# FrancisTheCat/raytracing_c

Hardware: AMD Instinct MI355X
Metric: Mray/s (higher is better)
Workload: dtype f32; 1 GPU; helmet.glb 1920x1080, 256 spp, 8 bounces (BASELINE.json configs[2]); partition=single GPU

## Files before the change

### include/rt_hip_diag.h

```cpp
#ifndef RT_HIP_DIAG_H
#define RT_HIP_DIAG_H

#include "rt_hip.h"

#ifdef __cplusplus
extern "C" {
#endif

extern void rt_diag_set_tokens(void *disney_proc, void *debug_proc, void *background_proc);

extern void rt_diag_multi_fault(i32 no_peer, i32 failing_slot);

extern int  rt_set_pipeline(i32 pipeline);
extern i32  rt_get_pipeline(void);
extern void rt_set_wavefront_capacity(i64 records);

extern int rt_get_ledger(u64 *out, i32 n);
extern int rt_get_wave_times(u64 *out, i32 max_waves);
extern i64 rt_diag_device_bytes_live(void);
extern int rt_diag_release_staging(void);
extern RT_Device_Scene *rt_diag_cached_scene(Scene const *scene);


extern int rt_test_math(i32 op, i32 n, f32 const *x, f32 const *y, f32 *out);
// ... 4 lines not shown
extern int rt_test_encode_sweep(u64 out[260]);
extern int rt_test_group_sum(i32 group, i32 n_waves, u64 const *in, u8 const *valid, u64 *out);
extern int rt_test_sky_add_group(void);
extern int rt_test_node_order(i32 n, u32 const *t_min, u8 const *cand, u32 *out);

extern int rt_test_trace(RT_Device_Scene *dscene, i32 n, f32 const *rays,
                         f32 *out_t, i32 *out_tri, f32 *out_uv);

extern int rt_test_trace_stream(RT_Device_Scene *dscene, i32 n, f32 const *rays, f32 const *pyramid, i32 exit_lanes, i32 mode,
                                f32 *out_t, i32 *out_tri, f32 *out_uv, u64 visits[2]);

extern int rt_test_tile_order(i32 n_tiles, u32 const *cost, u32 *order);

extern int rt_test_texture(RT_Device_Scene *dscene, i32 tex, i32 n, f32 const *uv, f32 *out_rgb);


#define RT_TEST_SHARED_TAPS 4
extern int rt_test_shade(RT_Device_Scene *dscene, i32 mode, i32 n, i32 const *tri, f32 const *in, u32 const *state_in,
                         f32 *out, u32 *state_out, i32 *terminate, i32 *textured);
extern int rt_test_shade_hit(RT_Device_Scene *dscene, i32 mode, i32 max_bounces, i32 n, i32 const *tri, f32 const *hit, f32 const *ray,
                             f32 const *carry, u32 const *state_in, i32 const *bounce_in, f32 *out, u32 *out_words);
extern int rt_test_feature_hit(RT_Device_Scene *dscene, i32 n, i32 const *tri, f32 const *hit, f32 const *ray, f32 *out, i32 *flag);
extern int rt_test_brdf(i32 n, f32 const *params, f32 const *in_dir, u32 const *state_in, f32 *out_dir, f32 *brdf, u32 *state_out);
extern int rt_test_background(RT_Device_Scene *dscene, i32 mode, i32 n, f32 const *dir, f32 *rgb);
extern int rt_test_primary_ray(Camera const *camera, i32 width, i32 height, i32 n, i32 const *xys, f32 *rays);

#ifdef __cplusplus
}
#endif

#endif
```

### raytracing_c_amd/csrc/rt_dev.hip.h

```cpp
#ifndef RT_DEV_HIP_H
#define RT_DEV_HIP_H

#include <hip/hip_runtime.h>
#include <stdint.h>

#include "rt_device.h"
#include "../../include/rt_math.h"

#define RT_BLOCK_WAVES 4
#define RT_BLOCK_THREADS (RT_BLOCK_WAVES * 64)

struct Ray3 {
  rt_v3 o, d;
  float inv_x, inv_y, inv_z;
  bool  fast;
};

__device__ __forceinline__ rt_v3 slab_bias3(const Ray3 &r) {
#ifdef RT_MATH_NO_FMA
  return rt_v3_make(0.0f, 0.0f, 0.0f);
#else
  float px, py, pz;
  asm volatile("v_mul_f32 %0, %1, %2" : "=v"(px) : "v"(r.o.x), "v"(r.inv_x));
  asm volatile("v_mul_f32 %0, %1, %2" : "=v"(py) : "v"(r.o.y), "v"(r.inv_y));
// ... 638 lines not shown
  if (POW24_LDS) p = rt_pow24_poly(b) * *reinterpret_cast<const float *>(reinterpret_cast<const char *>(rt_pow24_lds) + (((uint32_t)as_i(b) >> 21) & 28u));
  else p = rt_pow24_core(b);
  if (!(b >= 0x1p-5f && b < 2.0f)) p = rt_powf(b, 2.4f);
  return p;
#else
  const float b = __builtin_fmaf(r, c, q);
  const float t = __builtin_amdgcn_fmed3f(2.4f * rt_logf(b), -87.0f, 87.0f);
  const float p = rt_expf(t);
  return (b > 0.0f) ? p : 0.0f;
#endif
}
template <bool POW24_LDS = false>
__device__ __forceinline__ rt_v3 srgb_to_linear_tex(rt_v3 v) {
  return rt_v3_make(srgb_to_linear_tex1<POW24_LDS>(v.x), srgb_to_linear_tex1<POW24_LDS>(v.y), srgb_to_linear_tex1<POW24_LDS>(v.z));
}

__device__ __forceinline__ float bg_coord_u(float t) { return rt_madd(t, 1.0f / (2.0f * RT_PI), 0.5f); }
__device__ __forceinline__ float bg_coord_v(float t) { return rt_madd(-t, 1.0f / RT_PI, 0.5f); }
template <class PT>
__device__ __forceinline__ rt_v3 background_lookup(const PT &P, rt_v3 dir) {
  float u = bg_coord_u(atan2_dev(dir.z, dir.x));
  float v = bg_coord_v(asin_dev(dir.y));
  return srgb_to_linear_tex<Pow24InLds<PT>::value>(tex_bilinear<false>(P, P.bg_texture, u, v));
}


__device__ __forceinline__ float pow5(float m) { return m * m * m * m * m; }
__device__ __forceinline__ float luminance(rt_v3 x) { return rt_v3_dot(x, rt_v3_make(0.2126f, 0.7152f, 0.0722f)); }

__device__ __forceinline__ float ggx_D(float roughness, float NoH) {
  float a2 = roughness * roughness;
  float d = rt_madd(NoH * NoH, rt_madd(a2, a2, -1.0f), 1.0f);
  return a2 / (RT_PI * (d * d));
}

__device__ __forceinline__ float smith_G(float NDotV, float alpha2) {
  float a = alpha2 * alpha2;
  float b = NDotV * NDotV;
  return (2.0f * NDotV) / (NDotV + sqrt_dev(rt_madd(-a, b, a + b)));
}

__device__ __forceinline__ rt_v3 cosine_hemisphere(uint32_t &rng) {
  float angle = rt_rand_f32(&rng) * 2.0f * RT_PI;
  float distance = sqrt_dev(rt_rand_f32(&rng));
  float s, c;
  rt_sincosf(angle, &s, &c);
// ... 905 lines not shown
  const RT_DTexture *textures;
  const uint32_t *texels;
  int32_t bg_texture, max_bounces;
};

template <class SPT, class ARGS>
__device__ __forceinline__ void shade_params(SPT &SP, const ARGS A, const bool with_materials) {
  SP.tris = with_materials ? A->tris : nullptr; SP.mats = with_materials ? A->mats : nullptr;
  SP.textures = A->textures; SP.texels = A->texels;
  SP.bg_texture = A->bg_texture; SP.max_bounces = A->max_bounces;
}

struct ShadeParamsLds : ShadeParams {};
template <> struct Pow24InLds<ShadeParamsLds> { static constexpr bool value = RT_MATH_POW24 != 0; };

struct ShadeParamsShared : ShadeParams {};
struct ShadeParamsLdsShared : ShadeParamsLds {};
template <> struct SharedTaps<ShadeParamsShared> { static constexpr bool value = true; };
template <> struct SharedTaps<ShadeParamsLdsShared> { static constexpr bool value = true; };
template <> struct Pow24InLds<ShadeParamsLdsShared> { static constexpr bool value = RT_MATH_POW24 != 0; };
template <bool SHARED_TAPS> struct PathShadeParams { typedef ShadeParamsLds type; };
template <> struct PathShadeParams<true> { typedef ShadeParamsLdsShared type; };

struct PrimaryParams {
  float cam[3][4];
  float focal_length, inv_width, inv_height, aspect;
};
template <class CAM, class ARGS>
__device__ __forceinline__ void primary_params(PrimaryParams &PP, const CAM S, const ARGS A) {
#pragma unroll
  for (int i = 0; i < 3; i++)
#pragma unroll
    for (int j = 0; j < 4; j++) PP.cam[i][j] = S->cam[i][j];
  PP.focal_length = S->focal_length; PP.inv_width = A->inv_width; PP.inv_height = A->inv_height; PP.aspect = A->aspect;
}

#include "rt_tile.hip.h"

#endif
```

### raytracing_c_amd/csrc/rt_device.h

```cpp
#ifndef RT_DEVICE_H
#define RT_DEVICE_H

#include <stdint.h>

#define RT_NODE_F4   12
#define RT_LEAF_F4   18
#define RT_TRI_F4     7
#define RT_MAT_F4     9
#define RT_MAT_FLOATS 36
#define RT_MAX_DEPTH  8

#define RT_LDS_BYTES            (160 * 1024)
#define RT_LDS_NODE_BYTES       208
#define RT_LDS_TABLE_BYTES      64
#define RT_LDS_PERM_LEVEL_BYTES 256
#define RT_LDS_ACC_TILE_BYTES   1536

#define RT_MAT_DISNEY 0
#define RT_MAT_DEBUG  1

#define RT_TILE      8
#define RT_TILE_PIX  64

#define RT_PARK_RECORD_DWORDS (18 * 128)
enum {
  RT_CNT_PATHS = 0, RT_CNT_RAYS, RT_CNT_NODES, RT_CNT_LEAVES, RT_CNT_SHADES, RT_CNT_BG, RT_CNT_TEXTURED,
  RT_CNT_SKIPPED_ROOT,
  RT_CNT_LEDGER,
  RT_CNT_LEAFLESS = 136,
  RT_CNT_FUSED_ROOT,
  RT_CNT_TRIANGLELESS,
  RT_N_COUNTERS
};
#define RT_CNT_LEDGER_SLOTS (RT_CNT_LEAFLESS - RT_CNT_LEDGER)



typedef struct {
  uint32_t offset;
  int32_t  width, height, stride;
} RT_DTexture;
#define RT_TEX_TILE_INDEX(x, y, tpr) ((((y) >> 2) * (tpr) + ((x) >> 2)) * 16 + (((y) & 3) << 2) + ((x) & 3))

typedef struct RT_KView {
  float    cam[3][4];
  float    focal_length;
  uint32_t seed;
  uint32_t pad[2];
} RT_KView;

typedef struct {
  const float    *nodes;
  const float    *leaves;
  const float    *tris;
  const float    *mats;
  const RT_DTexture *textures;
  const uint32_t *texels;
  int32_t depth;
  int32_t last_row_offset;
  int32_t bg_texture;
  int32_t n_nodes;
  float cam[3][4];
  float focal_length;
  float inv_width, inv_height, aspect;
  int32_t width, height, samples, max_bounces;
// ... 15 lines not shown
  uint32_t *tile_next;
  uint32_t *open_groups;
  int32_t n_tiles;
  int32_t chunk_shift;
  int32_t n_chunks_tile;
  int32_t n_sample_blocks;
  int32_t drain_thresh;
  int32_t grab_max;
  uint32_t *park;
  int32_t short_div;
  int32_t pyr_nodes;
  uint32_t *wf_hit0;
  uint32_t *wf_hit;
  uint32_t *wf_ray[2];
  uint32_t *wf_cnt_hit0, *wf_cnt_hit, *wf_cnt_ray[2];
  uint32_t *wf_ctl;
  int32_t wf_soft_chunks;
  int32_t wf_bounce;
  int32_t wf_n_waves;
  const RT_KView *views;
  int32_t n_views;
  int32_t tiles_per_view;
  int32_t pixels_per_view;
} RT_KParams;

typedef struct {
  const float *rays;
  const float *t_max;
  float       *hits;
  uint8_t     *flags;
  uint32_t    *head;
  unsigned long long *counters;
  int32_t      n;
  int32_t      grab;
  int32_t      exit_lanes;
} RT_QParams;
enum { RT_QCNT_RAYS = 0, RT_QCNT_HITS, RT_QCNT_NODES, RT_QCNT_LEAVES, RT_QUERY_COUNTERS };
#define RT_HIT_DWORDS     22

typedef struct {
  unsigned long long *sums;
  uint32_t    *head;
  int32_t      n_units;
  int32_t      grab;
  int32_t      tiles_x;
  int32_t      shift;
// ... 39 lines not shown
```

### raytracing_c_amd/csrc/rt_diag.cpp

```cpp

#include "rt_host.h"

#include <cmath>
#include <vector>

#include "../../include/rt_math.h"
#include "../../include/rt_hip_diag.h"

#ifndef RT_DIAG_VARIANTS
#error rt_diag.cpp belongs to the diagnostic library only (-DRT_DIAG_VARIANTS)
#endif

extern "C" {
int rt_launch_test_math(int op, int n, const float *x, const float *y, float *out, hipStream_t stream);
int rt_launch_test_rcp_sweep(unsigned long long *counts, hipStream_t stream);
int rt_launch_test_srgb_sweep(unsigned long long *counts, hipStream_t stream);
int rt_launch_test_env_sweep(int which, uint32_t seed, unsigned long long *counts, hipStream_t stream);
int rt_launch_test_quantize_sweep(unsigned long long *counts, hipStream_t stream);
int rt_launch_test_encode_sweep(unsigned long long *counts, hipStream_t stream);
int rt_launch_test_sky_add_group(void);
int rt_launch_test_group_sum(int group, int n_waves, const unsigned long long *in, const unsigned char *valid, unsigned long long *out,
                              hipStream_t stream);
int rt_launch_test_node_order(int n, const uint32_t *t_min, const unsigned char *cand, uint32_t *out, hipStream_t stream);
int rt_launch_test_trace(const RT_KParams *P, int n, const float *rays, float *out_t, int *out_tri, float *out_uv,
                         hipStream_t stream);
int rt_launch_test_trace_stream(const RT_KParams *P, int n, const float *rays, const float *pyr, int exit_lanes, int n_blocks,
                                int smem_bytes, float *out_t, int *out_tri, float *out_uv, unsigned long long *visits,
                                hipStream_t stream);
int rt_launch_test_texture(const RT_KParams *P, int tex, int n, const float *uv, float *out, hipStream_t stream);
int rt_launch_test_shade(const RT_KParams *P, int lds, int n, const int *tri, const float *in, const uint32_t *state_in, float *out,
                         uint32_t *state_out, int *terminate, int *textured, hipStream_t stream);
int rt_launch_test_shade_hit(const RT_KParams *P, int mode, int n, const int *tri, const float *hit, const float *ray, const float *carry,
                             const uint32_t *state_in, const int *bounce_in, float *out, uint32_t *iout, hipStream_t stream);
int rt_launch_test_feature_hit(const RT_KParams *P, int n, const int *tri, const float *hit, const float *ray, float *out, int *flag,
                               hipStream_t stream);
int rt_launch_test_brdf(int n, const float *params, const float *in_dir, const uint32_t *state_in, float *out_dir, float *brdf,
                        uint32_t *state_out, hipStream_t stream);
int rt_launch_test_background(const RT_KParams *P, int lds, int n, const float *dir, float *rgb, hipStream_t stream);
int rt_launch_test_primary_ray(const RT_KParams *P, int n, const int *xys, float *rays, hipStream_t stream);
int rt_wf_launch_camera(const RT_KParams *P, int n_blocks, int geometry, int smem_bytes, hipStream_t stream);
int rt_wf_launch_trace(const RT_KParams *P, int n_blocks, int geometry, int smem_bytes, hipStream_t stream);
int rt_wf_launch_shade(const RT_KParams *P, int n_blocks, int first, hipStream_t stream);
}

std::atomic<int>            g_pipeline{0};
static std::atomic<int64_t> g_wf_cap_records{(int64_t)96 << 20};

extern "C" int rt_set_pipeline(i32 pipeline) {
  if (pipeline != 0 && pipeline != 1) return rt_fail("rt_set_pipeline: %d is not 0 (tile stream) or 1 (wavefront)", pipeline);
  g_pipeline.store(pipeline);
  return 0;
}
extern "C" i32 rt_get_pipeline(void) { return g_pipeline.load(); }
extern "C" void rt_set_wavefront_capacity(i64 records) {
  if (records >= 1024) g_wf_cap_records.store(records);
}

extern "C" void rt_diag_set_tokens(void *disney, void *debug, void *background) {
  if (disney) g_tok_disney = (Shader_Proc)disney;
  if (debug) g_tok_debug = (Shader_Proc)debug;
  if (background) g_tok_background = (Background_Proc)background;
// ... 479 lines not shown
  if (ensure_device(D) != 0) return -1;
  if (n <= 0 || !params || !in_dir || !state_in || !out_dir || !brdf || !state_out) return rt_fail("rt_test_brdf: bad arguments");
  DevMem<float> dp, di, dout, db;
  DevMem<uint32_t> ds0, ds1;
  HIP_TRY(dp.grow((size_t)n * 8));
  HIP_TRY(di.grow((size_t)n * 3));
  HIP_TRY(dout.grow((size_t)n * 3));
  HIP_TRY(db.grow((size_t)n * 4));
  HIP_TRY(ds0.grow((size_t)n));
  HIP_TRY(ds1.grow((size_t)n));
  HIP_TRY(hipMemcpy(dp, params, (size_t)n * 32, hipMemcpyHostToDevice));
  HIP_TRY(hipMemcpy(di, in_dir, (size_t)n * 12, hipMemcpyHostToDevice));
  HIP_TRY(hipMemcpy(ds0, state_in, (size_t)n * 4, hipMemcpyHostToDevice));
  int rc = rt_launch_test_brdf(n, dp, di, ds0, dout, db, ds1, nullptr);
  if (rc == 0) rc = (int)hipMemcpy(out_dir, dout, (size_t)n * 12, hipMemcpyDeviceToHost);
  if (rc == 0) rc = (int)hipMemcpy(brdf, db, (size_t)n * 16, hipMemcpyDeviceToHost);
  if (rc == 0) rc = (int)hipMemcpy(state_out, ds1, (size_t)n * 4, hipMemcpyDeviceToHost);
  if (rc != 0) return rt_fail("rt_test_brdf failed: %s", hipGetErrorString((hipError_t)rc));
  return 0;
}

extern "C" int rt_test_background(RT_Device_Scene *d, i32 mode, i32 n, f32 const *dir, f32 *rgb) {
  if (!d || n <= 0 || !dir || !rgb) return rt_fail("rt_test_background: bad arguments");
  if (mode != 0 && mode != 1) return rt_fail("rt_test_background: mode %d is not 0 (ShadeParams) or 1 (ShadeParamsLds)", mode);
  if (!all_finite(dir, (size_t)n * 3)) return rt_fail("rt_test_background: non-finite direction");
  Device &D = *d->dev;
  std::lock_guard<std::mutex> lock(D.mutex);
  DeviceGuard guard(D);
  if (ensure_device(D) != 0) return -1;
  RT_KParams K;
  scene_only_kparams(&K, d);
  DevMem<float> dd, dout;
  HIP_TRY(dd.grow((size_t)n * 3));
  HIP_TRY(dout.grow((size_t)n * 3));
  HIP_TRY(hipMemcpy(dd, dir, (size_t)n * 12, hipMemcpyHostToDevice));
  int rc = rt_launch_test_background(&K, mode, n, dd, dout, nullptr);
  if (rc == 0) rc = (int)hipMemcpy(rgb, dout, (size_t)n * 12, hipMemcpyDeviceToHost);
  if (rc != 0) return rt_fail("rt_test_background failed: %s", hipGetErrorString((hipError_t)rc));
  return 0;
}

extern "C" int rt_test_primary_ray(Camera const *camera, i32 width, i32 height, i32 n, i32 const *xys, f32 *rays) {
  Device &D = dev0();
  std::lock_guard<std::mutex> lock(D.mutex);
  if (ensure_device(D) != 0) return -1;
  if (!camera || width < 1 || height < 1 || n <= 0 || !xys || !rays) return rt_fail("rt_test_primary_ray: bad arguments");
  RT_KParams K;
  memset(&K, 0, sizeof K);
// ... 15 lines not shown
```

### raytracing_c_amd/csrc/rt_host.h

```cpp
#pragma once

#include <hip/hip_runtime.h>

#include <algorithm>
#include <atomic>
#include <chrono>
#include <cstdarg>
#include <cstdio>
#include <cstdlib>
#include <cstring>
#include <condition_variable>
#include <mutex>
#include <thread>
#include <unordered_map>
#include <vector>

#include "../../include/rt_hip.h"
#include "rt_device.h"
#include "rt_mem.h"

extern "C" {
int rt_launch_path_kernel(const RT_KParams *P, int n_waves, int smem_bytes, int wg_waves, hipStream_t stream);
int rt_launch_prepare(int n_tiles, uint32_t *tile_next, uint32_t *open_groups, unsigned long long *counters, uint32_t *work_head,
                      uint32_t *cost_cur, const uint32_t *cost_prev, uint32_t *order, hipStream_t stream);
int rt_launch_resolve(int width, int height, int samples, int chunks_x, const int32_t *local_chunks, int n_local_chunks,
                      const unsigned long long *accum, uint8_t *tiles, uint8_t *image, float *linear,
                      hipStream_t stream);
int rt_launch_untile(int width, int height, int chunks_x, int n_chunks, const int32_t *owner_slot,
                     const uint8_t *all_tiles, uint8_t *image, hipStream_t stream);
int rt_launch_lightmap(const RT_KParams *P, const float *verts, int n_tris, int lw, int lh, int stride, int comp,
                       int samples, int *owner, uint8_t *pixels, hipStream_t stream);
int rt_launch_denoise(int width, int height, int src_stride, int src_comp, int dst_stride, int dst_comp,
                      const uint8_t *src, uint8_t *dst, hipStream_t stream);
int rt_launch_pack_texture(const uint8_t *raw, int width, int rows, int y0, int stride, int comp, uint32_t *out,
                           hipStream_t stream);
int rt_launch_query(const RT_KParams *P, const RT_QParams *Q, int any, int wg_waves, int n_blocks, int smem_bytes, hipStream_t stream);
int rt_launch_hit_attributes(const RT_KParams *P, int n, const float *rays, const float *hits, float *out, hipStream_t stream);
int rt_launch_features(const RT_KParams *P, const RT_FParams *F, int n_blocks, int smem_bytes, hipStream_t stream);
int rt_launch_features_resolve(int n_pixels, int samples, const unsigned long long *sums, float *coverage, float *albedo, float *normal,
                               float *position, hipStream_t stream);
int rt_launch_features_motion(const RT_KParams *P, const RT_FParams *F, const float *kept, unsigned long long *motion_sums, int n_blocks,
                              int smem_bytes, hipStream_t stream);
int rt_launch_motion_resolve(int n_pixels, int samples, const unsigned long long *sums, float *motion, hipStream_t stream);
int rt_launch_refit(int len, int depth, int n_internal, const void *d_src, const int *d_source_of_slot, float *d_block, float *d_nodes,
                    float *d_leaves, float *d_tris, unsigned char *d_populated, unsigned int *d_max_edge_bits, hipStream_t stream);
int rt_refit_check(Scene const *scene, Triangle_Slice src, i32 const *slot_of_source, i32 *source_of_slot);
int rt_launch_guided_pack(int n_pixels, int demodulate, RT_Frame frame, void *c0, void *g0, void *g1, hipStream_t stream);
int rt_launch_guided_filter(int width, int height, int step, float k_n, float k_p, float k_c, int last, int demodulate, const void *src,
                            void *dst, const void *g0, const void *g1, RT_Frame frame, float *out, uint8_t *image, hipStream_t stream);
int rt_launch_temporal(const RT_TParams *P, RT_Frame frame, const void *hist_in, void *hist_out, float *out, float *length,
                       uint8_t *image, hipStream_t stream);
int rt_launch_temporal_motion(const RT_TParams *P, RT_Frame frame, const float *motion, const void *hist_in, void *hist_out, float *out,
                              float *length, uint8_t *image, hipStream_t stream);
int rt_launch_temporal_pack(int n_pixels, const float *c, const float *len, const float *cov, const float *n, const float *w, void *hist,
                            hipStream_t stream);
int rt_launch_temporal_unpack(int n_pixels, const void *hist, float *c, float *len, float *cov, float *n, float *w, hipStream_t stream);
int rt_launch_temporal_moments(const RT_TParams *P, RT_Frame frame, const void *hist_in, void *hist_out, float *out, float *length,
                               uint8_t *image, const void *mom_in, void *mom_out, hipStream_t stream);
// ... 275 lines not shown
  DevMem<uint32_t>    tile_next;
  int32_t             tile_next_n = 0;
  DevMem<uint32_t>    park;
  DevMem<uint32_t>    cost[2];
  DevMem<uint32_t>    order;
  int32_t      sched_tiles = 0, sched_cur = 0;
  bool         sched_valid = false;
  uint64_t     sched_key = 0;
  DevMem<RT_KView>    views;
  PinnedMem<RT_KView> views_host;
  DevEvent            views_copied;
  ChunkListStage      list;
};

#pragma GCC visibility pop

struct RT_Device_Scene {
  Device      *dev = nullptr;
  DevMem<float>       nodes, leaves, tris, mats;
  DevMem<float>       kept_leaves;
  bool                has_kept = false;
  DevMem<RT_DTexture> textures;
  DevMem<uint32_t>    texels;
  int32_t      depth = 0, last_row_offset = 0, bg_texture = -1, n_nodes = 0;
  int32_t      n_triangles = 0, n_materials = 0, n_textures = 0;
  int64_t      bytes = 0;
  float        max_edge = 0.0f;
  bool         boxes_ordered = true;
  std::vector<float> mats_host;
  bool         shared_taps = false;
  uint64_t     stamp = 0;
  std::vector<const void *> mat_ptrs;
  std::vector<int32_t>      mat_first_tri;
  std::vector<FpBlock>      fp_blocks;
  uint64_t                  full_fp = 0;
  std::unordered_map<uint64_t, int> mat_map;
  std::vector<const Image *>        tex_sources;
  std::vector<RT_DTexture>          tex_descs;
  LaunchState ls[RT_LAUNCH_STATES + 2];
  DevMem<uint32_t>    wf_hit0, wf_hit, wf_ray[2];
  DevMem<uint32_t>    wf_cnt;
  DevMem<uint32_t>    wf_ctl;
  PinnedMem<uint32_t> wf_ctl_host;
  int64_t             wf_soft0 = 0, wf_hard0 = 0, wf_ray_chunks = 0, wf_hit_chunks = 0;
  int32_t             wf_waves = 0;
};
// ... 94 lines not shown
```

### raytracing_c_amd/csrc/rt_kernels.hip

```cpp

#include "rt_dev.hip.h"


#ifdef RT_LEDGER
#define RT_LEDGER_WAVES 8192
__device__ uint32_t g_ledger[RT_LEDGER_WAVES * RT_LEDGER_ROW];
__global__ void rt_ledger_reduce_kernel(unsigned long long *counters) {
  const int slot = threadIdx.x;
  if (slot >= LG_N || slot >= RT_LEDGER_ROW) return;
  unsigned long long sum = 0ull;
  for (int w = 0; w < RT_LEDGER_WAVES; w++) sum += g_ledger[w * RT_LEDGER_ROW + slot];
  counters[RT_CNT_LEDGER + slot] = sum;
}
#endif

template <int WAVES, bool LDSN, int MIN_WAVES_PER_SIMD, bool SHORT_DIV, bool VIEWS, bool SHARED_TAPS>
__global__ __launch_bounds__(WAVES * 64, MIN_WAVES_PER_SIMD) void rt_path_kernel_stream(RT_KParams P) {
  extern __shared__ float4 smem[];
  const int lane = threadIdx.x & 63;
  const int wave = threadIdx.x >> 6;
  const int n_lds = LDSN ? P.n_lds_nodes : 0;
  const float4 *lds_nodes = smem;
  const WaveLds L = wave_lds(smem, n_lds, P.depth, wave);
  unsigned long long *acc = L.acc;
// ... 80 lines not shown
    LGT1(LG_CYC_TILE);

    int   pix = 0, bounce = 0;
    uint32_t rng = 0;
    Ray3  ray;
    ray_setup(ray, rt_v3_make(0, 0, 0), rt_v3_make(0, 0, 1));
    rt_v3 tint = rt_v3_make(1, 1, 1), emis = rt_v3_make(0, 0, 0);
    TravState T = RT_TRAV_IDLE;

    bool tile_open = true;
    TileUnits U;
    tile_units_init(U, queue_open);
    int  n_parked = 0;
    uint32_t *park = cold_args()->park;

    if ((tile_root_miss || n_list > 0) && cold_args()->max_bounces > 0) {
      RT_KArgs A = cold_args();
      typename CamSrc<VIEWS>::type S;
      if constexpr (VIEWS) S = vrec; else S = A;
      const int width = A->width, height = A->height, sample_first = A->sample_first, sample_end = A->sample_end;
      const uint32_t n_sb = (uint32_t)A->n_sample_blocks, gmax = (uint32_t)A->grab_max;
      PrimaryParams PP;
      primary_params(PP, S, A);
      ShadeParamsLds SP;
      shade_params(SP, A, false);
      uint32_t *tile_next = A->tile_next, *open_groups = A->open_groups;
      uint32_t n_sky = 0;
      const uint32_t *list = leafless_list(smem, pyr_off, ll_levels);
      const uint32_t list_entry = (n_list > 1 && lane_now() < n_list) ? list[RT_LL_ENTRY + (lane_now() & 31)] : 0u;
      for (;;) {
        if (U.c_next >= U.c_end) {
          if (U.u_cur + 1u < U.u_end) {
            U.u_cur += 1u;
          } else {
            uint32_t u0 = 0;
            if (lane == 0) u0 = atomicAdd(&tile_next[tile_idx], U.grab);
            u0 = (uint32_t)__builtin_amdgcn_readfirstlane((int)u0);
            if (u0 >= n_chunks_tile) { tile_open = false; break; }
            U.u_cur = u0;
            U.u_end = u0 + U.grab < n_chunks_tile ? u0 + U.grab : n_chunks_tile;
            if (U.u_end == n_chunks_tile && lane == 0) atomicSub(&open_groups[tile_idx >> 6], 1u);
            if (t_wave_start) t_last_grab = __builtin_amdgcn_s_memrealtime();
            LG(LG_GRAB_X, 1);
            const uint32_t left = n_chunks_tile - U.u_end;
            U.grab = left >= 8u * gmax ? gmax : (left >= 8u && gmax >= 2u ? 2u : 1u);
            U.took_any = true;
          }
          unit_decode(U, tile_x0, tile_y0, shift, unit_paths, n_sb, sample_first, width, height);
// ... 35 lines not shown
            const Ray3 &r = rs[q];
            const int nx = (as_i(r.inv_x) >> 31) & 96, ny = (as_i(r.inv_y) >> 31) & 96, nz = (as_i(r.inv_z) >> 31) & 96;
            const rt_v3 bs = slab_bias3(r);
            uint32_t entered = valid[q] ? 1u : 0u;
            int i = 1;
            if (q > 0) e = (uint32_t)__builtin_amdgcn_readlane((int)list_entry, 1);
            do {
              const char *cb = reinterpret_cast<const char *>(lds_nodes) + (e & 0xFFFFFu);
              const float t = slab_entry_ordered(r, bs, cb, 0, nx, ny, nz, RT_INF);
              const uint32_t in = ((entered >> ((e >> 20) & 31u)) & 1u) & (t < RT_INF ? 1u : 0u);
              entered |= in << i;
              const uint32_t n_in = (uint32_t)__popcll(__ballot(in != 0u));
              if (e & RT_LL_GROUP) w_leaves += n_in;
              else w_nodes += n_in;
              i += 1;
              e = (uint32_t)__builtin_amdgcn_readlane((int)list_entry, i);
            } while ((int)e < 0);
          }
        }
#pragma unroll
        for (int q = 0; q < RT_SKY_PATHS; q++) {
          unsigned long long qr = 0ull, qg = 0ull, qb = 0ull;
          if (valid[q]) {
            const rt_v3 bg = background_lookup(SP, dirs[q]);
            const rt_v3 radiance = rt_v3_mul_add(bg, rt_v3_make(1, 1, 1), rt_v3_make(0, 0, 0));
            qr = accum_quantize_dev(radiance.x); qg = accum_quantize_dev(radiance.y); qb = accum_quantize_dev(radiance.z);
          }
          tile_add_samples_grouped(smem, acc_off, U.c_pix0 + pxs[q], U.c_end >= 2 * RT_SKY_ADD_GROUP, valid[q], qr, qg, qb);
          nv += (uint32_t)__popcll(__ballot(valid[q]));
        }
        w_paths += nv; w_rays += nv; w_nodes += nv; w_bgs += nv;
        n_sky += nv;
        LG(LG_SKY_X, 1); LG(LG_SKY_L, nv);
        U.c_next += take;
        LGT1(LG_CYC_SKY);
        LGM("sky_end");
      }
      if (n_sky != 0u && lane == 0) atomicAdd(cold_args()->counters + (tile_root_miss ? RT_CNT_SKIPPED_ROOT : RT_CNT_LEAFLESS), (unsigned long long)n_sky);
      if (n_sky != 0u && (__ballot((list_entry & RT_LL_GROUP) != 0u) & ~1ull) != 0ull && lane == 0)
        atomicAdd(cold_args()->counters + RT_CNT_TRIANGLELESS, (unsigned long long)n_sky);
    }

    for (;;) {
      {
        LGT0();
        LGM("s_begin");
        LG(LG_S_ITER, 1);
// ... 559 lines not shown
  hipLaunchKernelGGL(rt_untile_kernel, dim3((n + 255) / 256), dim3(256), 0, stream, width, height, chunks_x,
                     n_chunks, owner_slot, all_tiles, image);
  return (int)hipGetLastError();
}

__global__ void rt_pack_texture_kernel(const uint8_t *raw, int width, int rows, int y0, int stride, int comp, uint32_t *out) {
  size_t i = (size_t)blockIdx.x * blockDim.x + threadIdx.x;
  if (i >= (size_t)width * rows) return;
  int yl = (int)(i / width), x = (int)(i % width);
  const uint8_t *p = raw + ((size_t)yl * stride + x) * comp;
  const int y = y0 + yl;
  const size_t o = (size_t)RT_TEX_TILE_INDEX(x, y, (width + 3) >> 2);
  out[o] = (uint32_t)p[0] | ((uint32_t)p[1] << 8) | ((uint32_t)p[2] << 16) | 0xFF000000u;
}

extern "C" int rt_launch_pack_texture(const uint8_t *raw, int width, int rows, int y0, int stride, int comp, uint32_t *out,
                                      hipStream_t stream) {
  size_t n = (size_t)width * rows;
  hipLaunchKernelGGL(rt_pack_texture_kernel, dim3((unsigned)((n + 255) / 256)), dim3(256), 0, stream, raw, width, rows, y0, stride,
                     comp, out);
  return (int)hipGetLastError();
}

template <int WAVES, bool ANY>
__global__ __launch_bounds__(WAVES * 64, 1) void rt_query_kernel(RT_KParams P, RT_QParams Q) {
  extern __shared__ float4 smem[];
  const int lane = threadIdx.x & 63;
  const int wave = threadIdx.x >> 6;
  const int n_lds = P.n_lds_nodes;
  lds_load_nodes<WAVES * 64>(smem, P.nodes, n_lds);
  __syncthreads();
  const int leaf_level = P.depth - 1;
  const TravWave W = {smem, smem, wave_perm(smem, n_lds, perm_stack_f4(P.depth), wave), n_lds, 0, 0, leaf_level, lane};
  int  next = 0, end = 0;
  bool drained = false;

  int   idx = 0;
  Ray3  ray;
  ray_setup(ray, rt_v3_make(0, 0, 0), rt_v3_make(0, 0, 1));
  uint32_t w_nodes = 0, w_leaves = 0, w_rays = 0, w_hits = 0;
  TravState T = RT_TRAV_IDLE;
  for (;;) {
    w_rays += (uint32_t)__popcll(__ballot(T.phase == PH_HIT || T.phase == PH_MISS));
    w_hits += (uint32_t)__popcll(__ballot(T.phase == PH_HIT));
    if (T.phase == PH_HIT || T.phase == PH_MISS) {
      if (ANY) Q.flags[idx] = T.phase == PH_HIT ? 1 : 0;
// ... 90 lines not shown
```

### raytracing_c_amd/csrc/rt_residency.cpp

```cpp

#include "rt_host.h"

void free_device_scene(RT_Device_Scene *d) {
  if (!d) return;
  if (d->dev) {
    for (FrameLane &F : d->dev->lanes)
      if (F.busy && F.d == d) {
        if (F.stream) (void)hipStreamSynchronize(F.stream);
        F.d = nullptr;
      }
    for (LaunchState &L : d->ls)
      if (L.counters && d->dev->last_counters == L.counters) d->dev->last_counters = nullptr;
  }
  delete d;
}

template <typename T>
static int upload(DevMem<T> &dst, const std::vector<T> &src, int64_t *bytes) {
  HIP_TRY(dst.grow(src.size()));
  if (!src.empty()) HIP_TRY(hipMemcpy(dst, src.data(), src.size() * sizeof(T), hipMemcpyHostToDevice));
  *bytes += (int64_t)dst.bytes();
  return 0;
}

// ... 6 lines not shown

static int texture_index(Image const *img, TexturePool &pool) {
  if (!img) return -1;
  auto it = pool.map.find(img);
  if (it != pool.map.end()) return it->second;
  if (img->pixel_type != PT_u8 || img->components < 3 || img->width <= 0 || img->height <= 0 || !img->pixels.data ||
      img->stride < img->width ||
      img->pixels.len < (isize)img->stride * img->height * img->components) {
    return -2;
  }
  RT_DTexture t;
  t.offset = (uint32_t)pool.texels;
  t.width = (int32_t)img->width;
  t.height = (int32_t)img->height;
  t.stride = (int32_t)((img->width + 3) / 4);
  pool.texels += (size_t)t.stride * (size_t)((img->height + 3) / 4) * 16;
  int idx = (int)pool.descs.size();
  pool.descs.push_back(t);
  pool.sources.push_back(img);
  pool.map[img] = idx;
  return idx;
}

static int upload_textures(const TexturePool &pool, DevMem<uint32_t> &d_texels, int64_t *bytes) {
  HIP_TRY(d_texels.grow(pool.texels));
  *bytes += (int64_t)d_texels.bytes();
  size_t max_raw = 0;
  for (const Image *img : pool.sources) {
    size_t raw = (size_t)img->stride * img->height * img->components;
    if (raw > max_raw) max_raw = raw;
  }
  if (max_raw == 0) return 0;
  DevMem<uint8_t> stage;
  HIP_TRY(stage.grow(max_raw));
  int rc = 0;
  for (size_t k = 0; k < pool.sources.size() && rc == 0; k++) {
    const Image *img = pool.sources[k];
    size_t raw = (size_t)img->stride * img->height * img->components;
    rc = (int)hipMemcpy(stage, img->pixels.data, raw, hipMemcpyHostToDevice);
    if (rc == 0) rc = rt_launch_pack_texture(stage, (int)img->width, (int)img->height, 0, (int)img->stride, (int)img->components,
                                             d_texels + pool.descs[k].offset, nullptr);
    if (rc == 0) rc = (int)hipDeviceSynchronize();
  }
  if (rc != 0) return rt_fail("texture upload failed: %s", hipGetErrorString((hipError_t)rc));
  return 0;
}

static inline uint64_t mix64(uint64_t h, uint64_t v) {
  h ^= v;
  h *= 0x9E3779B97F4A7C15ull;
  return h ^ (h >> 29);
}

static uint64_t hash_bytes(uint64_t seed, const void *data, size_t n, size_t stride_words = 1) {
  const unsigned char *b = (const unsigned char *)data;
  uint64_t h0 = seed ^ 0x243F6A8885A308D3ull, h1 = seed ^ 0x13198A2E03707344ull;
  uint64_t h2 = seed ^ 0xA4093822299F31D0ull, h3 = seed ^ 0x082EFA98EC4E6C89ull;
  size_t words = n / 8, i = 0;
  const size_t step = 4 * stride_words;
  for (; i + step <= words; i += step) {
    uint64_t w0, w1, w2, w3;
    memcpy(&w0, b + 8 * i, 8);
    memcpy(&w1, b + 8 * (i + stride_words), 8);
    memcpy(&w2, b + 8 * (i + 2 * stride_words), 8);
// ... 319 lines not shown
    leaf_tile_max_edge(&leaves[(size_t)g * 72], max_edge);
  }

  std::vector<float> nodes;
  bool boxes_ordered = true;
  if (scene->bvh.depth > 0) {
    const float *src = (const float *)scene->bvh.nodes.data;
    nodes.assign(src, src + (size_t)scene->bvh.nodes.len * 48);
    boxes_ordered = node_boxes_ordered(nodes.data(), (size_t)scene->bvh.nodes.len);
  }

  int bg = texture_index((Image const *)scene->background.data, pool);
  if (bg < 0) { rt_fail("rt_scene_upload: background Image is unusable (need PT_u8, >= 3 components, pixels.len >= stride*height*components)"); return nullptr; }

  RT_Device_Scene *d = new RT_Device_Scene();
  d->dev = &D;
  if (d->ls[0].counters.grow(RT_N_COUNTERS) != hipSuccess || d->ls[0].work_head.grow(16) != hipSuccess) {
    rt_fail("rt_scene_upload: out of device memory");
    free_device_scene(d);
    return nullptr;
  }
  if (upload(d->nodes, nodes, &d->bytes) || upload(d->leaves, leaves, &d->bytes) ||
      upload(d->tris, tris, &d->bytes) || upload(d->mats, mats, &d->bytes) ||
      upload(d->textures, pool.descs, &d->bytes) || upload_textures(pool, d->texels, &d->bytes)) {
    free_device_scene(d);
    return nullptr;
  }
  d->depth = (int32_t)scene->bvh.depth;
  d->last_row_offset = (int32_t)scene->bvh.last_row_offset;
  d->bg_texture = bg;
  d->n_nodes = (int32_t)scene->bvh.nodes.len;
  d->n_triangles = n;
  d->max_edge = max_edge;
  d->boxes_ordered = boxes_ordered;
  d->n_materials = (int32_t)(mats.size() / RT_MAT_FLOATS);
  d->mats_host = mats;
  refresh_shared_taps(d);
  d->n_textures = (int32_t)pool.descs.size();
  d->mat_ptrs = mat_ptrs;
  d->mat_first_tri = mat_first_tri;
  d->mat_map = mat_map;
  d->tex_sources = pool.sources;
  d->tex_descs = pool.descs;
  d->stamp = scene_stamp(scene, d->mat_ptrs, d->mat_first_tri);
  return d;
}

// ... 154 lines not shown
      if ((const void *)(uintptr_t)(kv.first / 2u) != d->mat_ptrs[k]) continue;
      float row[RT_MAT_FLOATS];
      build_material_row(m, ta, tn, tm, te, (int)(kv.first & 1u), d->tex_descs, row);
      HIP_TRY(hipMemcpy(d->mats + (size_t)kv.second * RT_MAT_FLOATS, row, sizeof row, hipMemcpyHostToDevice));
      memcpy(&d->mats_host[(size_t)kv.second * RT_MAT_FLOATS], row, sizeof row);
      any = true;
    }
    if (any) refresh_shared_taps(d);
    return any ? 1 : 0;
  }
  for (size_t t = 0; t < d->tex_sources.size(); t++) {
    const Image *img = d->tex_sources[t];
    const RT_DTexture &desc = d->tex_descs[t];
    if (img->width != desc.width || img->height != desc.height || img->components < 3 || img->pixel_type != PT_u8) continue;
    const size_t row_bytes = (size_t)img->stride * img->components;
    if (!range_in(begin, bytes, img->pixels.data, row_bytes * img->height, &off)) continue;
    const size_t r0 = off / row_bytes, r1 = (off + bytes + row_bytes - 1) / row_bytes;
    DevMem<uint8_t> stage;
    HIP_TRY(stage.grow((r1 - r0) * row_bytes));
    HIP_TRY(hipMemcpy(stage, (const unsigned char *)img->pixels.data + r0 * row_bytes, (r1 - r0) * row_bytes, hipMemcpyHostToDevice));
    uint32_t *tex_base = d->texels + desc.offset;
    int rc = rt_launch_pack_texture(stage, (int)img->width, (int)(r1 - r0), (int)r0, (int)img->stride,
                                    (int)img->components, tex_base, nullptr);
    if (rc == 0) rc = (int)hipDeviceSynchronize();
    if (rc != 0) return rt_fail("rt_scene_touch: texture rows: %s", hipGetErrorString((hipError_t)rc));
    return 1;
  }
  return 0;
}

static bool fp_block_holds(const FpBlock &b, const void *begin, size_t bytes) {
  const uintptr_t r0 = (uintptr_t)begin, r1 = r0 + bytes, b0 = (uintptr_t)b.begin, b1 = b0 + b.bytes;
  return b.begin && r0 < b1 && b0 < r1;
}

extern "C" int rt_scene_touch(Scene const *scene, void const *begin, size_t bytes) {
  if (!scene || !begin || bytes == 0) return rt_fail("rt_scene_touch: NULL scene or empty range");
  std::vector<FpBlock> now;
  scene_fingerprint_blocks(scene, now);
  int dropped = 0;
  for (int i = 0; i < RT_MAX_DEVICES; i++) {
    Device &D = g_devs[i];
    std::lock_guard<std::mutex> lock(D.mutex);
    auto it = D.scene_cache.find(scene);
    if (it == D.scene_cache.end()) continue;
    DeviceGuard guard(D);
// ... 65 lines not shown
extern "C" int rt_scene_verify(Scene const *scene) {
  if (!scene) return -1;
  {
    Device &D = dev0();
    std::lock_guard<std::mutex> lock(D.mutex);
    if (D.scene_cache.find(scene) == D.scene_cache.end()) return -1;
  }
  const uint64_t now = scene_fingerprint(scene);
  return drop_stale_copies(scene, now, 0) == 0 ? 1 : 0;
}

void scene_only_kparams(RT_KParams *K, RT_Device_Scene *d) {
  memset(K, 0, sizeof *K);
  K->nodes = d->nodes;
  K->leaves = d->leaves;
  K->tris = d->tris;
  K->mats = d->mats;
  K->textures = d->textures;
  K->texels = d->texels;
  K->depth = d->depth;
  K->last_row_offset = d->last_row_offset;
  K->bg_texture = d->bg_texture;
  K->n_nodes = d->n_nodes;
}

RT_Device_Scene *cached_scene_locked(Device &D, Scene const *scene, float *stamp_ms, float *upload_ms) {
  if (!scene) { rt_fail("render: scene is NULL"); return nullptr; }
  const double t0 = now_ms();
  auto it = D.scene_cache.find(scene);
  if (it != D.scene_cache.end()) {
    RT_Device_Scene *d = it->second;
    const bool same = d->stamp == scene_stamp(scene, d->mat_ptrs, d->mat_first_tri);
    if (stamp_ms) *stamp_ms = (float)(now_ms() - t0);
    if (same) return d;
    free_device_scene(d);
    D.scene_cache.erase(it);
  }
  const double t1 = now_ms();
  RT_Device_Scene *d = upload_scene_locked(D, scene);
  if (d) {
    D.scene_cache[scene] = d;
    scene_fingerprint_blocks(scene, d->fp_blocks);
    d->full_fp = fp_fold(d->fp_blocks);
  }
  if (upload_ms) *upload_ms = (float)(now_ms() - t1);
  return d;
// ... 30 lines not shown
```

Baseline: 24440 Mray/s.

## Add padded float copy of background for sky-path bilinear lookups

At scene upload, builds a float4 copy of the background texture with one extra padding column and row, and uses it in the sky-path kernel. Four texels are read directly and interpolated without the tiled u8 unpacking and wrap handling. This is meant to cut per-sample decode and addressing cost for rays that miss the geometry, at the price of extra device memory (16 bytes per texel) and more memory bandwidth per fetch. Only the leafless sky path uses the new lookup; other background lookups are unchanged.

Result: faster. 24710 Mray/s, median of 6 (+1.1%).

```diff
diff --git a/include/rt_hip_diag.h b/include/rt_hip_diag.h
--- a/include/rt_hip_diag.h
+++ b/include/rt_hip_diag.h
@@ -50,6 +50,7 @@
                              f32 const *carry, u32 const *state_in, i32 const *bounce_in, f32 *out, u32 *out_words);
 extern int rt_test_feature_hit(RT_Device_Scene *dscene, i32 n, i32 const *tri, f32 const *hit, f32 const *ray, f32 *out, i32 *flag);
 extern int rt_test_brdf(i32 n, f32 const *params, f32 const *in_dir, u32 const *state_in, f32 *out_dir, f32 *brdf, u32 *state_out);
+#define RT_TEST_BG_IMAGE 8
 extern int rt_test_background(RT_Device_Scene *dscene, i32 mode, i32 n, f32 const *dir, f32 *rgb);
 extern int rt_test_primary_ray(Camera const *camera, i32 width, i32 height, i32 n, i32 const *xys, f32 *rays);
 
diff --git a/raytracing_c_amd/csrc/rt_dev.hip.h b/raytracing_c_amd/csrc/rt_dev.hip.h
--- a/raytracing_c_amd/csrc/rt_dev.hip.h
+++ b/raytracing_c_amd/csrc/rt_dev.hip.h
@@ -684,6 +684,31 @@
   float u = bg_coord_u(atan2_dev(dir.z, dir.x));
   float v = bg_coord_v(asin_dev(dir.y));
   return srgb_to_linear_tex<Pow24InLds<PT>::value>(tex_bilinear<false>(P, P.bg_texture, u, v));
+}
+
+struct BgTexel { float r, g, b, pad; };
+template <class PT>
+__device__ __forceinline__ rt_v3 background_lookup_image(const PT &P, rt_v3 dir) {
+  const float tx = tex_wrap_fract<false>(bg_coord_u(atan2_dev(dir.z, dir.x)));
+  const float ty = tex_wrap_fract<false>(bg_coord_v(asin_dev(dir.y)));
+  typedef const RT_DTexture __attribute__((address_space(4))) CT;
+  CT *tp = (CT *)(unsigned long long)(P.textures + P.bg_texture);
+  const int width = tp->width, height = tp->height;
+  const float px = tx * (float)width;
+  const float py = ty * (float)height;
+  int u = (int)px, v = (int)py;
+  if (u > width - 1) u = width - 1;
+  if (v > height - 1) v = height - 1;
+  const float a = px - (float)u;
+  const float b = py - (float)v;
+  const uint32_t row = (uint32_t)P.bg_pitch * (uint32_t)sizeof(BgTexel);
+  const uint32_t o = (uint32_t)(v * P.bg_pitch + u) * (uint32_t)sizeof(BgTexel);
+  const char *base = reinterpret_cast<const char *>(P.bg_image);
+  const BgTexel *r0 = reinterpret_cast<const BgTexel *>(base + o), *r1 = reinterpret_cast<const BgTexel *>(base + (o + row));
+  const BgTexel q00 = r0[0], q10 = r0[1], q01 = r1[0], q11 = r1[1];
+  const rt_v3 c0 = rt_v3_lerp(rt_v3_make(q00.r, q00.g, q00.b), rt_v3_make(q10.r, q10.g, q10.b), a);
+  const rt_v3 c1 = rt_v3_lerp(rt_v3_make(q01.r, q01.g, q01.b), rt_v3_make(q11.r, q11.g, q11.b), a);
+  return srgb_to_linear_tex<Pow24InLds<PT>::value>(rt_v3_lerp(c0, c1, b));
 }
 
 
@@ -1635,6 +1660,19 @@
 template <bool SHARED_TAPS> struct PathShadeParams { typedef ShadeParamsLds type; };
 template <> struct PathShadeParams<true> { typedef ShadeParamsLdsShared type; };
 
+struct BgImageParams {
+  const RT_DTexture *textures;
+  const float *bg_image;
+  int32_t bg_texture, bg_pitch;
+};
+template <class ARGS>
+__device__ __forceinline__ void bg_image_params(BgImageParams &BP, const ARGS A) {
+  BP.textures = A->textures; BP.bg_image = A->bg_image;
+  BP.bg_texture = A->bg_texture; BP.bg_pitch = A->bg_pitch;
+}
+struct BgImageParamsLds : BgImageParams {};
+template <> struct Pow24InLds<BgImageParamsLds> { static constexpr bool value = RT_MATH_POW24 != 0; };
+
 struct PrimaryParams {
   float cam[3][4];
   float focal_length, inv_width, inv_height, aspect;
diff --git a/raytracing_c_amd/csrc/rt_device.h b/raytracing_c_amd/csrc/rt_device.h
--- a/raytracing_c_amd/csrc/rt_device.h
+++ b/raytracing_c_amd/csrc/rt_device.h
@@ -41,6 +41,9 @@
   int32_t  width, height, stride;
 } RT_DTexture;
 #define RT_TEX_TILE_INDEX(x, y, tpr) ((((y) >> 2) * (tpr) + ((x) >> 2)) * 16 + (((y) & 3) << 2) + ((x) & 3))
+
+#define RT_BG_TEXEL_FLOATS 4
+#define RT_BG_IMAGE_MAX_BYTES 0xFFFFFFFFull
 
 typedef struct RT_KView {
   float    cam[3][4];
@@ -102,6 +105,9 @@
   int32_t n_views;
   int32_t tiles_per_view;
   int32_t pixels_per_view;
+  const float *bg_image;
+  int32_t bg_pitch;
+  int32_t bg_pad;
 } RT_KParams;
 
 typedef struct {
diff --git a/raytracing_c_amd/csrc/rt_diag.cpp b/raytracing_c_amd/csrc/rt_diag.cpp
--- a/raytracing_c_amd/csrc/rt_diag.cpp
+++ b/raytracing_c_amd/csrc/rt_diag.cpp
@@ -36,7 +36,7 @@
                                hipStream_t stream);
 int rt_launch_test_brdf(int n, const float *params, const float *in_dir, const uint32_t *state_in, float *out_dir, float *brdf,
                         uint32_t *state_out, hipStream_t stream);
-int rt_launch_test_background(const RT_KParams *P, int lds, int n, const float *dir, float *rgb, hipStream_t stream);
+int rt_launch_test_background(const RT_KParams *P, int mode, int n, const float *dir, float *rgb, hipStream_t stream);
 int rt_launch_test_primary_ray(const RT_KParams *P, int n, const int *xys, float *rays, hipStream_t stream);
 int rt_wf_launch_camera(const RT_KParams *P, int n_blocks, int geometry, int smem_bytes, hipStream_t stream);
 int rt_wf_launch_trace(const RT_KParams *P, int n_blocks, int geometry, int smem_bytes, hipStream_t stream);
@@ -562,8 +562,8 @@
 
 extern "C" int rt_test_background(RT_Device_Scene *d, i32 mode, i32 n, f32 const *dir, f32 *rgb) {
   if (!d || n <= 0 || !dir || !rgb) return rt_fail("rt_test_background: bad arguments");
-  if (mode != 0 && mode != 1) return rt_fail("rt_test_background: mode %d is not 0 (ShadeParams) or 1 (ShadeParamsLds)", mode);
-  if (!all_finite(dir, (size_t)n * 3)) return rt_fail("rt_test_background: non-finite direction");
+  if ((mode & ~RT_TEST_BG_IMAGE) != 0 && (mode & ~RT_TEST_BG_IMAGE) != 1)
+    return rt_fail("rt_test_background: mode %d is not 0 (ShadeParams) or 1 (ShadeParamsLds), with or without RT_TEST_BG_IMAGE", mode);
   Device &D = *d->dev;
   std::lock_guard<std::mutex> lock(D.mutex);
   DeviceGuard guard(D);
diff --git a/raytracing_c_amd/csrc/rt_host.h b/raytracing_c_amd/csrc/rt_host.h
--- a/raytracing_c_amd/csrc/rt_host.h
+++ b/raytracing_c_amd/csrc/rt_host.h
@@ -34,6 +34,8 @@
                       const uint8_t *src, uint8_t *dst, hipStream_t stream);
 int rt_launch_pack_texture(const uint8_t *raw, int width, int rows, int y0, int stride, int comp, uint32_t *out,
                            hipStream_t stream);
+int rt_launch_pack_bg_image(const uint8_t *raw, int width, int height, int rows, int y0, int stride, int comp, float *out,
+                            hipStream_t stream);
 int rt_launch_query(const RT_KParams *P, const RT_QParams *Q, int any, int wg_waves, int n_blocks, int smem_bytes, hipStream_t stream);
 int rt_launch_hit_attributes(const RT_KParams *P, int n, const float *rays, const float *hits, float *out, hipStream_t stream);
 int rt_launch_features(const RT_KParams *P, const RT_FParams *F, int n_blocks, int smem_bytes, hipStream_t stream);
@@ -355,6 +357,7 @@
   bool                has_kept = false;
   DevMem<RT_DTexture> textures;
   DevMem<uint32_t>    texels;
+  DevMem<float>       bg_image;
   int32_t      depth = 0, last_row_offset = 0, bg_texture = -1, n_nodes = 0;
   int32_t      n_triangles = 0, n_materials = 0, n_textures = 0;
   int64_t      bytes = 0;
diff --git a/raytracing_c_amd/csrc/rt_kernels.hip b/raytracing_c_amd/csrc/rt_kernels.hip
--- a/raytracing_c_amd/csrc/rt_kernels.hip
+++ b/raytracing_c_amd/csrc/rt_kernels.hip
@@ -126,8 +126,8 @@
       const uint32_t n_sb = (uint32_t)A->n_sample_blocks, gmax = (uint32_t)A->grab_max;
       PrimaryParams PP;
       primary_params(PP, S, A);
-      ShadeParamsLds SP;
-      shade_params(SP, A, false);
+      BgImageParamsLds BP;
+      bg_image_params(BP, A);
       uint32_t *tile_next = A->tile_next, *open_groups = A->open_groups;
       uint32_t n_sky = 0;
       const uint32_t *list = leafless_list(smem, pyr_off, ll_levels);
@@ -209,7 +209,7 @@
         for (int q = 0; q < RT_SKY_PATHS; q++) {
           unsigned long long qr = 0ull, qg = 0ull, qb = 0ull;
           if (valid[q]) {
-            const rt_v3 bg = background_lookup(SP, dirs[q]);
+            const rt_v3 bg = background_lookup_image(BP, dirs[q]);
             const rt_v3 radiance = rt_v3_mul_add(bg, rt_v3_make(1, 1, 1), rt_v3_make(0, 0, 0));
             qr = accum_quantize_dev(radiance.x); qg = accum_quantize_dev(radiance.y); qb = accum_quantize_dev(radiance.z);
           }
@@ -815,6 +815,28 @@
   return (int)hipGetLastError();
 }
 
+__global__ void rt_pack_bg_image_kernel(const uint8_t *raw, int width, int height, int rows, int y0, int stride, int comp, float4 *out) {
+  const int pitch = width + 1;
+  size_t i = (size_t)blockIdx.x * blockDim.x + threadIdx.x;
+  if (i >= (size_t)pitch * rows) return;
+  int yl = (int)(i / pitch), x = (int)(i % pitch);
+  const int xs = x < width ? x : width - 1;
+  const uint8_t *p = raw + ((size_t)yl * stride + xs) * comp;
+  const int y = y0 + yl;
+  const rt_v3 c = texel_rgb((uint32_t)p[0] | ((uint32_t)p[1] << 8) | ((uint32_t)p[2] << 16));
+  const float4 t = make_float4(c.x, c.y, c.z, 0.0f);
+  out[(size_t)y * pitch + x] = t;
+  if (y == height - 1) out[(size_t)height * pitch + x] = t;
+}
+
+extern "C" int rt_launch_pack_bg_image(const uint8_t *raw, int width, int height, int rows, int y0, int stride, int comp, float *out,
+                                       hipStream_t stream) {
+  size_t n = (size_t)(width + 1) * rows;
+  hipLaunchKernelGGL(rt_pack_bg_image_kernel, dim3((unsigned)((n + 255) / 256)), dim3(256), 0, stream, raw, width, height, rows, y0,
+                     stride, comp, reinterpret_cast<float4 *>(out));
+  return (int)hipGetLastError();
+}
+
 template <int WAVES, bool ANY>
 __global__ __launch_bounds__(WAVES * 64, 1) void rt_query_kernel(RT_KParams P, RT_QParams Q) {
   extern __shared__ float4 smem[];
diff --git a/raytracing_c_amd/csrc/rt_residency.cpp b/raytracing_c_amd/csrc/rt_residency.cpp
--- a/raytracing_c_amd/csrc/rt_residency.cpp
+++ b/raytracing_c_amd/csrc/rt_residency.cpp
@@ -52,9 +52,15 @@
   return idx;
 }
 
-static int upload_textures(const TexturePool &pool, DevMem<uint32_t> &d_texels, int64_t *bytes) {
+static int upload_textures(const TexturePool &pool, DevMem<uint32_t> &d_texels, int bg, DevMem<float> &d_bg_image, int64_t *bytes) {
   HIP_TRY(d_texels.grow(pool.texels));
   *bytes += (int64_t)d_texels.bytes();
+  const size_t bg_texels = ((size_t)pool.descs[bg].width + 1) * ((size_t)pool.descs[bg].height + 1);
+  if (bg_texels * RT_BG_TEXEL_FLOATS * sizeof(float) > RT_BG_IMAGE_MAX_BYTES)
+    return rt_fail("rt_scene_upload: the background (%d x %d) is too large for its float copy", pool.descs[bg].width, pool.descs[bg].height);
+  if (d_bg_image.grow(bg_texels * RT_BG_TEXEL_FLOATS) != hipSuccess)
+    return rt_fail("rt_scene_upload: out of device memory for the float copy of the background (%zu bytes)", bg_texels * RT_BG_TEXEL_FLOATS * sizeof(float));
+  *bytes += (int64_t)d_bg_image.bytes();
   size_t max_raw = 0;
   for (const Image *img : pool.sources) {
     size_t raw = (size_t)img->stride * img->height * img->components;
@@ -70,6 +76,8 @@
     rc = (int)hipMemcpy(stage, img->pixels.data, raw, hipMemcpyHostToDevice);
     if (rc == 0) rc = rt_launch_pack_texture(stage, (int)img->width, (int)img->height, 0, (int)img->stride, (int)img->components,
                                              d_texels + pool.descs[k].offset, nullptr);
+    if (rc == 0 && (int)k == bg) rc = rt_launch_pack_bg_image(stage, (int)img->width, (int)img->height, (int)img->height, 0, (int)img->stride,
+                                                              (int)img->components, d_bg_image, nullptr);
     if (rc == 0) rc = (int)hipDeviceSynchronize();
   }
   if (rc != 0) return rt_fail("texture upload failed: %s", hipGetErrorString((hipError_t)rc));
@@ -435,7 +443,7 @@
   }
   if (upload(d->nodes, nodes, &d->bytes) || upload(d->leaves, leaves, &d->bytes) ||
       upload(d->tris, tris, &d->bytes) || upload(d->mats, mats, &d->bytes) ||
-      upload(d->textures, pool.descs, &d->bytes) || upload_textures(pool, d->texels, &d->bytes)) {
+      upload(d->textures, pool.descs, &d->bytes) || upload_textures(pool, d->texels, bg, d->bg_image, &d->bytes)) {
     free_device_scene(d);
     return nullptr;
   }
@@ -636,6 +644,8 @@
     uint32_t *tex_base = d->texels + desc.offset;
     int rc = rt_launch_pack_texture(stage, (int)img->width, (int)(r1 - r0), (int)r0, (int)img->stride,
                                     (int)img->components, tex_base, nullptr);
+    if (rc == 0 && (int)t == d->bg_texture) rc = rt_launch_pack_bg_image(stage, (int)img->width, (int)img->height, (int)(r1 - r0), (int)r0,
+                                                                         (int)img->stride, (int)img->components, d->bg_image, nullptr);
     if (rc == 0) rc = (int)hipDeviceSynchronize();
     if (rc != 0) return rt_fail("rt_scene_touch: texture rows: %s", hipGetErrorString((hipError_t)rc));
     return 1;
@@ -747,6 +757,8 @@
   K->last_row_offset = d->last_row_offset;
   K->bg_texture = d->bg_texture;
   K->n_nodes = d->n_nodes;
+  K->bg_image = d->bg_image;
+  K->bg_pitch = d->tex_descs[(size_t)d->bg_texture].width + 1;
 }
 
 RT_Device_Scene *cached_scene_locked(Device &D, Scene const *scene, float *stamp_ms, float *upload_ms) {
```
